# ctu-mrs/mrs_multirotor_simulator

Measured on NVIDIA B200. Metric: UAV-steps/s (RK4+control+collisions) at 1M UAVs, higher is better.
Workload: dtype f64

## Files before the change

mrs_multirotor_simulator_b200/csrc/api.cu:

```cuda
#include <dlfcn.h>
#include <nccl.h>

#include <algorithm>
#include <cmath>
#include <cstdarg>
#include <cstdio>
#include <cstring>
#include <functional>
#include <map>
#include <memory>
#include <string>
#include <type_traits>
#include <utility>
#include <vector>

#include "internal.h"
#include "params.h"

static thread_local char g_err[512] = "";

static int fail(int code, const char* fmt, ...) {
  va_list ap;
  va_start(ap, fmt);
  vsnprintf(g_err, sizeof(g_err), fmt, ap);
// ... 68 lines not shown

  int alloc(size_t count) {
    Mem m;
    if (Pinned) {
      CU(cudaHostAlloc(&m.p_, sizeof(T) * count, cudaHostAllocMapped));
    } else {
      CU(cudaMalloc(&m.p_, sizeof(T) * count));
    }
    m.cap_ = count;
    *this  = std::move(m);
    return MRSB_OK;
  }
  int grow(size_t need, size_t count, cudaStream_t stream) {
    if (need <= cap_) return MRSB_OK;
    Mem m;
    int rc = m.alloc(count);
    if (rc) return rc;
    if (p_) CU(cudaStreamSynchronize(stream));
    *this = std::move(m);
    return MRSB_OK;
  }

 private:
  void release() {
    if (p_) Pinned ? cudaFreeHost(p_) : cudaFree(p_);
  }
  T*     p_   = nullptr;
  size_t cap_ = 0;
};

struct ParamSet {
  mrsb_model_params      mp;
  mrsb_controller_params cp;
};

#define MAX_BUCKETS 8
struct Bucket {
  int64_t   slot0 = 0, count = 0;
  int       nm    = 0;
  int       pset  = -1;
  DevParams params{};
};

static_assert(std::is_trivially_copyable_v<DevState> && std::is_trivially_copyable_v<DevGrid> && std::is_trivially_copyable_v<PeerView> &&
              std::is_trivially_copyable_v<P2PCtl> && std::is_trivially_copyable_v<DevParams> && std::is_trivially_copyable_v<Bucket>);
struct GraphArgs {
  DevState s;
  DevGrid  grid;
  PeerView pv;
  P2PCtl   p2p;
  int32_t  crash, lists;
  double   rebounce;
  int32_t with_step, k_substeps, uniform_mode, any_moment, publish, n_buckets;
  double  dt;
  Bucket  buckets[MAX_BUCKETS];
};
static_assert(std::is_trivially_copyable_v<GraphArgs>);

struct Graph {
  cudaGraphExec_t exec = nullptr;
  int             own  = 0;
  GraphArgs       key{};

  Graph() = default;
  explicit Graph(const GraphArgs& a) { std::memcpy(&key, &a, sizeof(a)); }
  Graph(Graph&& o) noexcept { *this = std::move(o); }
  Graph& operator=(Graph&& o) noexcept {
    if (exec) cudaGraphExecDestroy(exec);
    exec = std::exchange(o.exec, nullptr), own = o.own;
    std::memcpy(&key, &o.key, sizeof(key));
    return *this;
  }
  ~Graph() {
    if (exec) cudaGraphExecDestroy(exec);
  }
  bool holds(const GraphArgs& a) const { return std::memcmp(&key, &a, sizeof(a)) == 0; }
};

struct mrsb_sim {
  int          device = 0;
  cudaStream_t stream = nullptr;
  DevState     ds{};
  DevGrid      grid{};
  Mem<int32_t> pairs;

  std::vector<ParamSet>      sets;
  std::map<std::string, int> set_index;
  std::vector<Mem<unsigned char>> mem;

  std::vector<int32_t>       pset_host;
  Mem<DevParams>             d_params;
  Mem<uint8_t>               d_takeoff0;
  int32_t*                   d_pset       = nullptr;
  bool                       params_dirty = true;

  Mem<char>    d_stage;
  Mem<int32_t> d_idx;

  int  uniform_mode = MRSB_INPUT_UNKNOWN;
  bool any_moment   = false;
  std::vector<Bucket>  buckets;
  std::vector<int32_t> perm_host, inv_host;
  int32_t*             d_perm = nullptr;
  int32_t*             d_inv  = nullptr;

  int    coll_enabled = 0, coll_crash = 0;
  double coll_rebounce = 0.0;

  double   filt_dt  = -1.0;
  uint32_t outputs  = MRSB_OUT_IMU | MRSB_OUT_POSITIONS;
  bool     iterate_without_input = true;
  double*  d_geom[2] = {nullptr, nullptr};

  ncclComm_t           comm    = nullptr;
  int                  n_ranks = 1, rank = 0;
  std::vector<int64_t> shard_begin_of, shard_count_of;
  bool                 equal_shards = true;

  bool                 p2p       = false;
  double*              gbuf[2]   = {nullptr, nullptr};
  uint32_t*            d_gbox[2] = {nullptr, nullptr};
  int64_t              pass_no   = 0;
  bool                 wrote_since_pass = false;
  std::vector<int32_t> pending_geom[2];
  PeerView             pv[2]{};
  PeerView             pv_local{};
  P2PCtl               p2pctl{};
// ... 1152 lines not shown
  if (h->p2p) {
    h->pass_no++;
    const int w         = write_buf(h);
    h->ds.gpos          = h->gbuf[w];
    h->ds.gbox          = h->d_gbox[w];
    h->ds.geom          = h->d_geom[w];
    h->wrote_since_pass = false;
    int rc              = apply_pending_geom(h, w);
    if (rc) return rc;
  }
  CU(cudaGetLastError());
  return MRSB_OK;
}

static int collide_local(mrsb_sim* h) {
  if (h->p2p && !h->wrote_since_pass) {
    h->n_launches += launch_publish_positions(h->ds, h->stream);
    h->wrote_since_pass = true;
  }
  if (h->lists_on) {
    int rc = before_list_pass(h);
    if (rc) return rc;
  } else {
    h->steps_since_pass = 0;
  }
  GraphArgs a;
  graph_args(h, false, 0.0, 0, &a);
  Graph& g       = h->pass[write_buf(h)];
  bool   graphed = !h->graph_failed && !getenv("MRSB_NO_GRAPH");
  if (graphed && !(g.exec && g.holds(a))) {
    g               = build_pass_graph(h, a);
    graphed         = g.exec != nullptr;
    h->graph_failed = !graphed;
  }
  if (graphed) {
    CU(cudaGraphLaunch(g.exec, h->stream));
    h->n_launches += g.own;
  } else if (a.lists) {
    h->n_launches += launch_collide_decide(a.grid, a.p2p, 1, cudaGraphConditionalHandle{}, 0, h->stream);
    h->rebuild_own = launch_collide_rebuild(a.s, a.grid, a.pv, h->stream);
    h->rebuild_own += launch_collide_check(a.s, a.grid, a.pv, a.crash, a.rebounce, 0, h->stream);
  } else {
    h->n_launches += launch_collide(a.s, a.grid, a.pv, a.p2p, a.crash, a.rebounce, h->stream);
  }
  return after_pass(h);
}

static int before_step(mrsb_sim* h, double dt, int32_t k_substeps) {
  if (k_substeps < 1) return fail(MRSB_ERR_INVALID, "k_substeps must be >= 1");
  int rc = flush_params(h);
  if (rc) return rc;
  rc = ensure_filt(h, dt);
  if (rc) return rc;
  if (h->p2p && *h->h_status.get()) return fail(MRSB_ERR_STATE, "peer hand-shake timed out (a rank stopped calling the collision pass)");
  return MRSB_OK;
}

int mrsb_make_step(mrsb_handle h, double dt, int32_t k_substeps) {
  GUARD(h);
  int rc = before_step(h, dt, k_substeps);
  if (rc) return rc;
  GraphArgs a;
  graph_args(h, true, dt, k_substeps, &a);
  h->n_launches += launch_step_buckets(a, h->stream, h->step_info);
  h->wrote_since_pass = true;
  h->n_steps += k_substeps;
  h->steps_since_pass++;
  CU(cudaGetLastError());
  return MRSB_OK;
}

static int before_collisions(mrsb_sim* h) {
  int rc = flush_params(h);
  if (rc) return rc;
  if (h->ds.n_global > h->ds.n && h->n_ranks <= 1) return fail(MRSB_ERR_STATE, "sharded handle without communicator");
  if (h->lists_on && (h->positions_touched || h->steps_since_pass != 1))
    CU(cudaMemcpyAsync(&h->grid.ctl->disp_max_bits, h->h_one.get() + 1, sizeof(uint32_t), cudaMemcpyHostToDevice, h->stream));
  return MRSB_OK;
}

int mrsb_handle_collisions(mrsb_handle h) {
  GUARD(h);
  if (!(h->coll_crash || h->coll_enabled)) return MRSB_OK;
  int rc = before_collisions(h);
  if (rc) return rc;
  rc = exchange_positions(h);
  if (rc) return rc;
  return collide_local(h);
}

int mrsb_handle_collisions_gathered(mrsb_handle h) {
  GUARD(h);
  if (!(h->coll_crash || h->coll_enabled)) return MRSB_OK;
  int rc = flush_params(h);
  if (rc) return rc;
  return collide_local(h);
}

static int run_tick_graph(mrsb_sim* h, double dt, int32_t k_substeps, bool* done) {
  *done = false;
  if (!h->lists_on || h->graph_failed || getenv("MRSB_NO_GRAPH")) return MRSB_OK;
  if (h->positions_touched || h->steps_since_pass != 0) return MRSB_OK;
  GraphArgs a;
  graph_args(h, true, dt, k_substeps, &a);
  Graph& g = h->tick[write_buf(h)];
  if (!g.holds(a)) {
    g = Graph(a);
    return MRSB_OK;
  }
  if (!g.exec) {
    g = build_pass_graph(h, a);
    if (!g.exec) {
      h->graph_failed = true;
      return MRSB_OK;
    }
  }
  h->wrote_since_pass = true;
  h->n_steps += k_substeps;
  h->list_passes++;
  CU(cudaGraphLaunch(g.exec, h->stream));
  h->n_launches += g.own;
  *done = true;
  return after_pass(h);
}

int mrsb_run(mrsb_handle h, double dt, int32_t k_substeps, int32_t n_ticks, int32_t with_collisions) {
  GUARD(h);
  const bool collide = with_collisions && (h->coll_crash || h->coll_enabled);
  for (int t = 0; t < n_ticks; t++) {
    if (collide) {
      int rc = before_step(h, dt, k_substeps);
      if (rc) return rc;
      bool done = false;
      rc        = run_tick_graph(h, dt, k_substeps, &done);
      if (rc) return rc;
      if (done) continue;
    }
    int rc = mrsb_make_step(h, dt, k_substeps);
    if (rc) return rc;
    if (collide) {
      rc = mrsb_handle_collisions(h);
      if (rc) return rc;
    }
  }
  return MRSB_OK;
}

int mrsb_get_state(mrsb_handle h, int64_t n, const int32_t* idx, double* x, double* v, double* R, double* omega, double* motor_rpm) {
  GUARD(h);
  int rc = MRSB_OK;
  if (x && !rc) rc = get_rows(h, h->ds.st, ST_ROWS, 0, 3, n, idx, x);
  if (v && !rc) rc = get_rows(h, h->ds.st, ST_ROWS, 3, 3, n, idx, v);
  if (R && !rc) rc = get_rows(h, h->ds.st, ST_ROWS, 6, 9, n, idx, R);
  if (omega && !rc) rc = get_rows(h, h->ds.st, ST_ROWS, 15, 3, n, idx, omega);
  if (motor_rpm && !rc) rc = get_rows(h, h->ds.rpm, MRSB_NM, 0, MRSB_NM, n, idx, motor_rpm);
  return rc;
}

int mrsb_get_v_prev(mrsb_handle h, int64_t n, const int32_t* idx, double* v_prev) {
  GUARD(h);
  return download(h, n, idx, sizeof(double) * 3 * size_t(n), v_prev, [&](const int32_t* d_idx, void* d_out) {
    return launch_gather_vprev(h->ds, n, d_idx, static_cast<double*>(d_out), h->stream);
  });
}
// ... 749 lines not shown
```

mrs_multirotor_simulator_b200/csrc/collide.cu:

```cuda
#include <algorithm>

#include "internal.h"

namespace {

#define DEV __device__ __forceinline__

#define NL_LIVE 0x80000000u
#define NL_CROWDED 0x40000000u

DEV unsigned long long now_ns() {
  unsigned long long t;
  asm volatile("mov.u64 %0, %globaltimer;" : "=l"(t));
  return t;
}
DEV void stamp(const DevGrid& g, int slot, unsigned long long value) {
  if (g.tl) g.tl[((g.ctl->n_passes - 1ull) % MRSB_TL_TICKS) * 8 + slot] = value;
}

DEV int cell_of(double v, double inv_cell) {
  return __double2int_rd(__dmul_rn(v, inv_cell));
}

DEV uint32_t row_hash(int cy, int cz) {
  uint32_t h = uint32_t(cy) * 0x9E3779B1u ^ (uint32_t(cz) * 0x85EBCA77u + 0x165667B1u);
  h ^= h >> 15;
  h *= 0x2C1B3C6Du;
  h ^= h >> 12;
  return h;
}

DEV unsigned long long enc(double v) {
  const unsigned long long b = (unsigned long long)__double_as_longlong(v);
  return (b >> 63) ? ~b : (b | 0x8000000000000000ull);
}
DEV double dec(unsigned long long e) {
  const unsigned long long b = (e >> 63) ? (e & 0x7fffffffffffffffull) : ~e;
  return __longlong_as_double((long long)b);
}
DEV float fdec(uint32_t e) {
  return __uint_as_float((e >> 31) ? (e & 0x7fffffffu) : ~e);
}

DEV int owner_of(const PeerView& pv, int64_t gj) {
  int r = 0;
  while (r + 1 < pv.n_ranks && gj >= pv.begin[r + 1]) r++;
  return r;
}
DEV void load_pos(const DevState& s, int64_t gj, double& x, double& y, double& z) {
  const double* p = s.gpos + 3 * gj;
  x = p[0], y = p[1], z = p[2];
}
struct Geom {
  double arm, prop, mass;
};
DEV Geom load_geom(const DevState& s, int64_t gj) {
  const double* p = s.geom + 4 * gj;
  Geom          g;
  g.arm = p[0], g.prop = p[1], g.mass = p[2];
  return g;
}

__global__ void box_reset_kernel(unsigned long long* aabb) {
  if (threadIdx.x < 3) aabb[threadIdx.x] = ~0ull;
  if (threadIdx.x >= 3 && threadIdx.x < 6) aabb[threadIdx.x] = 0ull;
}

__global__ void __launch_bounds__(256) box_kernel(const double* __restrict__ gpos, int64_t begin, int64_t n, unsigned long long* aabb) {
// ... 626 lines not shown
          hits &= hits - 1;
        }
      } else {
        int64_t last = -1;
        while (hits) {
          int64_t  best = INT64_MAX;
          uint32_t bc   = 0;
          for (uint32_t m = hits; m; m &= m - 1) {
            const uint32_t c  = uint32_t(__ffs(int(m)) - 1);
            const int64_t  gj = g.act_items[int64_t(c) * g.nl_ld + k];
            if (gj > last && gj < best) best = gj, bc = c;
          }
          if (best == INT64_MAX) break;
          process(bc);
          last = best;
          hits &= ~(1u << bc);
        }
      }
    }
  }
  const bool nz = nonzero(acc);
  if (live || nz) store_result(s, li, acc);
  else if (acc.crashed_me) s.flags[slot_of(s, li)] |= FLAG_CRASHED;
  if (nz != bool(word & NL_LIVE)) {
    const uint32_t nw = (word & ~NL_LIVE) | (nz ? NL_LIVE : 0u);
    g.nl_count[li]    = nw;
    g.nl_active[k].y  = nw;
  }
}

#ifndef MRSB_CHECK_THREADS
#define MRSB_CHECK_THREADS 256
#define MRSB_CHECK_MINB 4
#endif
__global__ void __launch_bounds__(MRSB_CHECK_THREADS, MRSB_CHECK_MINB) check_kernel(DevState s, DevGrid g, int crash_mode, double rebounce, int skip_if_rebuild) {
  if (skip_if_rebuild && g.ctl->rebuild) return;
  if (blockIdx.x == 0 && threadIdx.x == 0) stamp(g, 4, now_ns());
  const uint32_t n_active = g.ctl->n_active;
  for (uint32_t k = blockIdx.x * blockDim.x + threadIdx.x; k < n_active; k += gridDim.x * blockDim.x) {
    const uint2 e = g.nl_active[k];
    int32_t     first4[4];
#pragma unroll
    for (int u = 0; u < 4; u++) first4[u] = g.act_items[int64_t(u) * g.nl_ld + k];
    check_one(s, g, crash_mode, rebounce, k, int64_t(e.x), e.y, first4);
  }
}

__global__ void __launch_bounds__(32) decide_kernel(NlCtl* __restrict__ c, unsigned long long* __restrict__ pair_counter, double skin, int always,
                                                    cudaGraphConditionalHandle handle, int has_handle, P2PCtl p, unsigned long long* tl) {
  const uint32_t full = 0xffffffffu;
  const int      lane = threadIdx.x;
  unsigned long long* row = tl ? tl + (c->n_passes % MRSB_TL_TICKS) * 8 : nullptr;
  if (row && lane == 0) row[0] = now_ns();
  uint32_t                 bits  = c->disp_max_bits;
  const double             D_old = c->D_total;
  const uint32_t           force = c->force, valid = c->valid;
  const unsigned long long n_rebuilds = c->n_rebuilds, n_passes = c->n_passes;
  if (p.n_ranks > 1) {
    const unsigned long long epoch = c->epoch + 1ull;
    const int                slot  = int(epoch & 1ull);
    const bool               peer  = lane < p.n_ranks && lane != p.rank;
    volatile unsigned long long* theirs = peer ? p.peer_flags[lane] : nullptr;
    if (peer) theirs[p.n_ranks + 2 * p.rank + slot] = (unsigned long long)(always ? 0xFFFFFFFFu : bits);
    __threadfence_system();
    if (peer) theirs[p.rank] = epoch;
    if (row && lane == 0) row[1] = now_ns();
    uint32_t got = 0u;
    if (peer) {
      volatile const unsigned long long* mine = p.flags;
      const long long                    t0   = clock64();
      bool                               ok   = true;
      while (mine[lane] < epoch) {
        if (clock64() - t0 > p.budget) {
          *p.status = 1;
          ok        = false;
          break;
        }
        __nanosleep(32);
      }
      __threadfence_system();
      got = ok ? uint32_t(mine[p.n_ranks + 2 * lane + slot]) : 0xFFFFFFFFu;
    }
    bits = max(bits, __reduce_max_sync(full, got));
    if (lane == 0) c->epoch = epoch;
  }
  if (lane != 0) return;
  if (row) row[2] = now_ns();
  const double d       = __dsqrt_ru(double(__uint_as_float(bits)));
  double       D       = __dadd_ru(D_old, d);
  const bool   rebuild = always || force || !valid || !(__dmul_ru(2.0, D) <= skin);
  if (has_handle) cudaGraphSetConditional(handle, rebuild ? 1u : 0u);
  *pair_counter    = 0ull;
  c->disp_max_bits = 0u;
  if (rebuild) {
    D            = 0.0;
    c->force     = 0u;
    c->valid     = 1u;
    c->n_crowded = 0u;
    c->n_active  = 0u;
    c->n_rebuilds = n_rebuilds + 1ull;
  }
  if (row) row[5] = rebuild ? 1ull : 0ull;
  c->D_total  = D;
  c->rebuild  = rebuild ? 1u : 0u;
  c->n_passes = n_passes + 1ull;
}


__global__ void __launch_bounds__(256) nb_pack_kernel(DevState s, double* __restrict__ pos, double* __restrict__ vel) {
  const int64_t i = int64_t(blockIdx.x) * blockDim.x + threadIdx.x;
  if (i >= s.ld) return;
  const int64_t e = s.inv ? int64_t(s.inv[i]) : (i < s.n ? i : -1);
  if (e < 0) return;
#pragma unroll
  for (int c = 0; c < 3; c++) {
    pos[3 * e + c] = s.st[tix(ST_ROWS, c, i)];
    vel[3 * e + c] = s.st[tix(ST_ROWS, 3 + c, i)];
  }
}

DEV bool nb_before(double da, int32_t ja, double db, int32_t jb) { return da < db || (da == db && ja < jb); }

template <int K>
__global__ void __launch_bounds__(128) nb_query_kernel(DevGrid t, int64_t n, const double* __restrict__ pos, const double* __restrict__ vel, double r2,
                                                        int k, int32_t* __restrict__ idx_out, double* __restrict__ rows_out, int64_t stride,
                                                        int32_t* __restrict__ count_out) {
  const int64_t p = int64_t(blockIdx.x) * blockDim.x + threadIdx.x;
  if (p >= n) return;
  const double4 q = t.rec[p];
  const int64_t i = __double_as_longlong(q.w);
  double        bd[K];
  int32_t       bj[K];
#pragma unroll
  for (int u = 0; u < K; u++) bd[u] = __longlong_as_double(0x7FF0000000000000ll), bj[u] = INT32_MAX;
  int32_t cnt = 0;
  if (isfinite(q.x) && isfinite(q.y) && isfinite(q.z)) {
    const Stencil st = stencil_of(t, q.x, q.y, q.z);
    for (int a = 0; a < 4; a++) {
      for (uint32_t r = st.lo[a]; r < st.hi[a]; r++) {
        const double4 c  = t.rec[r];
        const double  d2 = nf_dist2(c.x, c.y, c.z, q.x, q.y, q.z);
        if (!(d2 < r2)) continue;
        const int32_t j = int32_t(__double_as_longlong(c.w));
        if (int64_t(j) == i || cell_of(c.y, t.inv_cell) != st.rcy[a] || cell_of(c.z, t.inv_cell) != st.rcz[a]) continue;
        cnt++;
        if (!nb_before(d2, j, bd[K - 1], bj[K - 1])) continue;
        bd[K - 1] = d2, bj[K - 1] = j;
#pragma unroll
        for (int u = K - 1; u > 0; u--) {
          if (nb_before(bd[u], bj[u], bd[u - 1], bj[u - 1])) {
            const double  td = bd[u];
            const int32_t tj = bj[u];
            bd[u] = bd[u - 1], bj[u] = bj[u - 1];
            bd[u - 1] = td, bj[u - 1] = tj;
          }
        }
      }
    }
// ... 143 lines not shown
```

mrs_multirotor_simulator_b200/csrc/internal.h:

```cpp
#pragma once
#include <cuda_runtime.h>
#include <stdint.h>

#include "../../include/mrsb.h"

#define MRSB_NM MRSB_MAX_MOTORS
#define MRSB_TILE 128

static __host__ __device__ __forceinline__ int64_t tix(int rows, int row, int64_t i) {
  return ((i >> 7) * rows + row) * MRSB_TILE + (i & (MRSB_TILE - 1));
}
#define ST_ROWS 18
#define VPREV_ROWS 3
#define F3_ROWS 3

#define FLAG_CRASHED 1u
#define FLAG_TAKEOFF 2u
#define FLAG_VPREV 4u
#define FLAG_HAD_INPUT 256u
#define FLAG_FF_VEL_HDG_RATE 16u
#define FLAG_FF_VEL_HDG 32u
#define FLAG_FF_ACC_HDG_RATE 64u
#define FLAG_FF_ACC_HDG 128u

// ... 38 lines not shown
  double*  initz;
  double*  cmd;
  double*  ff;
  uint32_t* flags;
  uint8_t*  mode;
  const int32_t* pset;
  const DevParams* params;
  double* geom;
  double*  gpos;
  int64_t  shard_begin;
  int64_t  n_global;
  uint32_t* gbox;
  int64_t   n_groups32;
  int32_t  n_ranks, rank;
  uint32_t opts;
  const int32_t* perm;
  const int32_t* inv;
  uint32_t* disp_max;
};

#define STEP_OPT_IMU 1u
#define STEP_OPT_GPOS 2u
#define STEP_OPT_NEED_INPUT 4u

#define MRSB_MAX_RANKS 16
struct PeerView {
  int32_t         n_ranks, rank;
  int64_t         begin[MRSB_MAX_RANKS + 1];
  const double*   pos[MRSB_MAX_RANKS];
  const uint32_t* box[MRSB_MAX_RANKS];
  const double*   geom[MRSB_MAX_RANKS];
};

struct P2PCtl {
  unsigned long long* const* peer_flags;
  unsigned long long*        flags;
  int32_t                    n_ranks, rank;
  int*                       status;
  long long                  budget;
};

#define MRSB_NL_CAP 8
#define MRSB_TL_TICKS 4096
struct NlCtl {
  uint32_t disp_max_bits;
  uint32_t force;
  uint32_t valid;
  uint32_t n_active;
  uint32_t n_crowded;
  uint32_t rebuild;
  double   D_total;
  unsigned long long n_rebuilds, n_passes, epoch ;
  unsigned long long write_all_until;
};

struct DevGrid {
  uint32_t  n_buckets;
  uint32_t  bits;
  double    inv_cell;
  double    reach;
  double    list_r2;
  double    skin;
  uint32_t* nl_count;
  int32_t*  nl_items;
  int64_t   nl_ld;
  uint2*    nl_active;
  int32_t*  act_items;
  NlCtl*    ctl;
  uint32_t* bucket;
  uint32_t* rank;
  uint32_t* count;
  uint32_t* begin;
  double4*  rec;
  unsigned long long* aabb;
  unsigned long long* scan_state;
  int32_t   scan_tiles;
  double4*  halo_rec;
  uint32_t* halo_bucket, *halo_rank;
  uint32_t* halo_n;
  uint32_t* halo_work;
  uint32_t* halo_work_n;
  int64_t   halo_cap;
  unsigned long long* tl;
  int32_t*  pairs;
  int64_t   pair_cap;
  unsigned long long* counters;
};

int launch_step(const DevState& s, const DevParams* uniform_params, double dt, int k_substeps, int uniform_mode, int uniform_nm, bool any_moment,
                cudaStream_t stream, int* info);
int launch_prep_params(DevParams* params, int n_sets, double dt, cudaStream_t stream);
int launch_collide(const DevState& s, const DevGrid& g, const PeerView& pv, const P2PCtl& p2p, int crash_mode, double rebounce, cudaStream_t stream);
int launch_collide_decide(const DevGrid& g, const P2PCtl& p2p, int always, cudaGraphConditionalHandle handle, int has_handle, cudaStream_t stream);
int launch_collide_rebuild(const DevState& s, const DevGrid& g, const PeerView& pv, cudaStream_t stream);
int launch_collide_check(const DevState& s, const DevGrid& g, const PeerView& pv, int crash_mode, double rebounce, int beside_rebuild, cudaStream_t stream);
int scan_tiles_for(int64_t n_items);
int launch_neighbours(const DevState& s, const DevGrid& t, double* pos, double* vel, double r2, int k, int32_t* idx, double* rows, int stride,
                      int32_t* count, cudaStream_t stream);
int launch_publish_positions(const DevState& s, cudaStream_t stream);

int launch_scatter_input(const DevState& s, int mode, int64_t n, const int32_t* idx_dev, const double* payload_dev, int stride, cudaStream_t stream);
int launch_input_rows(const DevState& s, int64_t n, const int32_t* idx_dev, const int32_t* modes_dev, const double* payload_dev, int stride,
                      int32_t* last_dev, cudaStream_t stream);
int launch_scatter_rows(double* dst, int rows_total, int row0, int rows, int64_t n, const int32_t* idx_dev, const double* payload_dev, int stride,
                        const int32_t* perm, cudaStream_t stream);
int launch_gather_rows(const double* src, int rows_total, int row0, int rows, int64_t n, const int32_t* idx_dev, double* out_dev, int stride,
                       const int32_t* perm, cudaStream_t stream);
int launch_flag_update(const DevState& s, int64_t n, const int32_t* idx_dev, uint32_t and_mask, uint32_t or_mask, cudaStream_t stream);
int launch_gather_u32(const uint32_t* src, int64_t n, const int32_t* idx_dev, uint32_t* out_dev, const int32_t* perm, cudaStream_t stream);
int launch_gather_u8(const uint8_t* src, int64_t n, const int32_t* idx_dev, int32_t* out_dev, const int32_t* perm, cudaStream_t stream);
int launch_set_mode(const DevState& s, int64_t n, const int32_t* idx_dev, int mode, cudaStream_t stream);
int launch_set_state_pos(const DevState& s, int64_t n, const int32_t* idx_dev, const double* xyz_dev, const double* hdg_dev, cudaStream_t stream);
int launch_respawn(const DevState& s, const uint8_t* takeoff0, int64_t n, const int32_t* idx_dev, const double* xyz_dev, const double* hdg_dev,
                   cudaStream_t stream);
int launch_respawn_masked(const DevState& s, const uint8_t* takeoff0, const uint8_t* mask_dev, const double* xyz_dev, const double* hdg_dev,
                          cudaStream_t stream);
#define SNAP_ROWS 88
int launch_snapshot_save(const DevState& s, double* rows, uint32_t* flags, uint8_t* mode, cudaStream_t stream);
int launch_snapshot_restore(const DevState& s, const double* rows, const uint32_t* flags, const uint8_t* mode, int64_t n, const int32_t* idx_dev,
                            const int32_t* src_dev, cudaStream_t stream);
int launch_snapshot_restore_masked(const DevState& s, const double* rows, const uint32_t* flags, const uint8_t* mode, const int32_t* src_dev,
                                   cudaStream_t stream);
int launch_stash_vprev(const DevState& s, int64_t n, const int32_t* idx_dev, cudaStream_t stream);
int launch_gather_vprev(const DevState& s, int64_t n, const int32_t* idx_dev, double* out_dev, cudaStream_t stream);
int launch_reset_pid(const DevState& s, int64_t n, const int32_t* idx_dev, int pid0, int n_pids, cudaStream_t stream);
int launch_timeout_input(const DevState& s, int64_t n, const int32_t* idx_dev, cudaStream_t stream);
int launch_gather_xyz(const double* xyz_dev, int64_t n, const int32_t* idx_dev, double* out_dev, cudaStream_t stream);
int launch_tracker_cmd(const DevState& s, int64_t n, const int32_t* idx_dev, const double* rows_dev, cudaStream_t stream);
int launch_observe(const DevState& s, int what, int64_t n, const int32_t* idx_dev, double* out_dev, int stride, cudaStream_t stream);
int launch_set_pset(int32_t* pset_dev, int64_t n, const int32_t* idx_dev, int64_t offset, const int32_t* values_dev, cudaStream_t stream);
int launch_set_geom(double* geom_dev, int64_t n, const int32_t* idx_dev, int64_t offset, const int32_t* pset_dev, const DevParams* params, cudaStream_t stream);
```

mrs_multirotor_simulator_b200/csrc/step_kernel.cu:

```cuda
#include <cstdlib>

#include "internal.h"

template <int NM_T>
void launch_step_nm(const DevState& s, const DevParams* uniform_params, double dt, int k_substeps, int uniform_mode, bool any_moment, cudaStream_t stream, int* info);

int launch_step(const DevState& s, const DevParams* uniform_params, double dt, int k_substeps, int uniform_mode, int uniform_nm, bool any_moment,
                cudaStream_t stream, int* info) {
  int scratch[4];
  if (!info) info = scratch;
  info[0] = info[1] = info[2] = info[3] = 0;
  if (s.n <= 0) return 0;
  switch (uniform_nm) {
    case 4:
      launch_step_nm<4>(s, uniform_params, dt, k_substeps, uniform_mode, any_moment, stream, info);
      break;
    case 6:
      launch_step_nm<6>(s, uniform_params, dt, k_substeps, uniform_mode, any_moment, stream, info);
      break;
    case 8:
      launch_step_nm<8>(s, uniform_params, dt, k_substeps, uniform_mode, any_moment, stream, info);
      break;
    default:
      launch_step_nm<0>(s, uniform_params, dt, k_substeps, uniform_mode, any_moment, stream, info);
      break;
  }
  return 1;
}

namespace {
__device__ __forceinline__ uint32_t fenc(float f) {
  const uint32_t b = __float_as_uint(f);
  return (b >> 31) ? ~b : (b | 0x80000000u);
}

__global__ void __launch_bounds__(256) publish_positions_kernel(DevState s) {
  const int64_t i      = int64_t(blockIdx.x) * blockDim.x + threadIdx.x;
  const bool    inside = i < s.n;
  double        x = 0.0, y = 0.0, z = 0.0;
  if (inside) {
    const int64_t slot = s.perm ? int64_t(s.perm[i]) : i;
    x          = s.st[tix(ST_ROWS, 0, slot)];
    y          = s.st[tix(ST_ROWS, 1, slot)];
    z          = s.st[tix(ST_ROWS, 2, slot)];
    double* gp = s.gpos + 3 * (s.shard_begin + i);
    gp[0]      = x;
    gp[1]      = y;
    gp[2]      = z;
  }
  if (s.gbox) {
    const uint32_t full = 0xffffffffu;
    uint32_t lo0 = inside ? fenc(__double2float_rd(x)) : 0xFFFFFFFFu, lo1 = inside ? fenc(__double2float_rd(y)) : 0xFFFFFFFFu,
             lo2 = inside ? fenc(__double2float_rd(z)) : 0xFFFFFFFFu;
    uint32_t hi0 = inside ? fenc(__double2float_ru(x)) : 0u, hi1 = inside ? fenc(__double2float_ru(y)) : 0u, hi2 = inside ? fenc(__double2float_ru(z)) : 0u;
    lo0 = __reduce_min_sync(full, lo0);
    lo1 = __reduce_min_sync(full, lo1);
    lo2 = __reduce_min_sync(full, lo2);
    hi0 = __reduce_max_sync(full, hi0);
    hi1 = __reduce_max_sync(full, hi1);
    hi2 = __reduce_max_sync(full, hi2);
    if ((threadIdx.x & 31) == 0 && i < s.n_groups32 * 32) {
      uint32_t* row = s.gbox + 6 * (i >> 5);
      row[0] = lo0, row[1] = lo1, row[2] = lo2, row[3] = hi0, row[4] = hi1, row[5] = hi2;
    }
  }
}

__global__ void prep_params_kernel(DevParams* params, int n_sets, double dt) {
  const int k = blockIdx.x * blockDim.x + threadIdx.x;
  if (k < n_sets) params[k].filt = exp(dt * params[k].neg_inv_tau);
}
}

int launch_prep_params(DevParams* params, int n_sets, double dt, cudaStream_t stream) {
  if (n_sets <= 0) return 0;
  prep_params_kernel<<<(n_sets + 127) / 128, 128, 0, stream>>>(params, n_sets, dt);
  return 1;
}

int launch_publish_positions(const DevState& s, cudaStream_t stream) {
// ... 5 lines not shown
```

mrs_multirotor_simulator_b200/csrc/step_kernel.cuh:

```cuda
#include <cstdlib>
#include <type_traits>

#pragma once
#include "internal.h"

namespace {

#define DEV __device__ __forceinline__

DEV double rsqrt_fast(double x) {
  double y;
  asm("rsqrt.approx.ftz.f64 %0, %1;" : "=d"(y) : "d"(x));
  const double t = x * y;
  const double e = fma(-t, y, 1.0);
  const double p = fma(0.375, e, 0.5);
  return fma(y * e, p, y);
}
DEV double rcp_fast(double b) {
  double r;
  asm("rcp.approx.ftz.f64 %0, %1;" : "=d"(r) : "d"(b));
  const double e = fma(-b, r, 1.0);
  const double p = fma(e, e, e);
  return fma(r, p, r);
}
DEV double sqrt_fast(double x) {
  if (x > 1e-290 && x < 1e300) return x * rsqrt_fast(x);
  return sqrt(x);
}
DEV unsigned expo(double v) { return unsigned(__double2hiint(v)) & 0x7ff00000u; }

struct Vec3 {
  double x, y, z;
};
DEV Vec3 mk(double x, double y, double z) {
  Vec3 r;
  r.x = x;
  r.y = y;
  r.z = z;
  return r;
}
DEV Vec3   operator+(Vec3 a, Vec3 b) { return mk(a.x + b.x, a.y + b.y, a.z + b.z); }
DEV Vec3   operator-(Vec3 a, Vec3 b) { return mk(a.x - b.x, a.y - b.y, a.z - b.z); }
DEV Vec3   operator*(Vec3 a, double s) { return mk(a.x * s, a.y * s, a.z * s); }
DEV double dot(Vec3 a, Vec3 b) { return fma(a.x, b.x, fma(a.y, b.y, a.z * b.z)); }
DEV Vec3   cross(Vec3 a, Vec3 b) { return mk(fma(a.y, b.z, -(a.z * b.y)), fma(a.z, b.x, -(a.x * b.z)), fma(a.x, b.y, -(a.y * b.x))); }
DEV Vec3   fma3(Vec3 a, double s, Vec3 b) { return mk(fma(a.x, s, b.x), fma(a.y, s, b.y), fma(a.z, s, b.z)); }
DEV Vec3 normalized(Vec3 a) {
  const double z = dot(a, a);
  if (z > 1e-290 && z < 1e300) return a * rsqrt_fast(z);
  if (z > 0.0) return a * (1.0 / sqrt(z));
  return a;
}
DEV unsigned expo3(Vec3 a) { return max(expo(a.x), max(expo(a.y), expo(a.z))); }
DEV bool isnan3(Vec3 a) { return (a.x != a.x) | (a.y != a.y) | (a.z != a.z); }
DEV Vec3 nan0(Vec3 a) { return mk(a.x != a.x ? 0.0 : a.x, a.y != a.y ? 0.0 : a.y, a.z != a.z ? 0.0 : a.z); }

struct Rot {
// ... 663 lines not shown
  if ((threadIdx.x & 31) == 0 && disp_bits > *reinterpret_cast<volatile uint32_t*>(s.disp_max)) atomicMax(s.disp_max, disp_bits);
}

template <int NM_T, int MODE_T, bool ONE>
__global__ void __launch_bounds__(MRSB_STEP_THREADS, MRSB_STEP_MINB(ONE, MODE_T))
    uav_step_kernel(DevState s, double dt, double inv_dt, int k_sub, int any_moment) {
  const int64_t tile = blockIdx.x;
  TileIn        in;
  in.st   = s.st + (tile * ST_ROWS) * MRSB_TILE + threadIdx.x;
  in.rpm  = s.rpm + (tile * MRSB_NM) * MRSB_TILE + threadIdx.x;
  in.pid  = s.pid + (tile * PID_ROWS) * MRSB_TILE + threadIdx.x;
  in.cmd  = s.cmd + (tile * CMD_ROWS) * MRSB_TILE + threadIdx.x;
  in.fext = s.fext + (tile * F3_ROWS) * MRSB_TILE + threadIdx.x;
  const int64_t i = min(tile * MRSB_TILE + threadIdx.x, s.n - 1);
  uint32_t disp_bits = 0u;
  step_uav<NM_T, MODE_T, ONE>(s, in, tile, s.flags[i], nullptr, s.pset[s.shard_begin + (s.inv ? int64_t(s.inv[i]) : i)], dt, inv_dt, k_sub, any_moment, disp_bits,
                              [] {});
  report_displacement(s, disp_bits);
}

template <int NM_T, int MODE_T>
struct Img {
  static constexpr int  pid_lo   = MODE_T == MRSB_POSITION_CMD ? 0 : MODE_T >= MRSB_VELOCITY_HDG_RATE_CMD ? 3 : MODE_T >= MRSB_ATTITUDE_CMD ? 6 : MODE_T >= MRSB_ATTITUDE_RATE_CMD ? 9 : 12;
  static constexpr int  cmd_rows = MODE_T == MRSB_ACTUATOR_CMD ? NM_T : MODE_T == MRSB_ATTITUDE_CMD ? 10 : MODE_T == MRSB_TILT_HDG_RATE_CMD ? 5 : 4;
  static constexpr bool hdg      = MODE_T == MRSB_POSITION_CMD || MODE_T == MRSB_VELOCITY_HDG_CMD || MODE_T == MRSB_ACCELERATION_HDG_CMD;
  static constexpr int  ST       = 0;
  static constexpr int  RPM      = ST + ST_ROWS;
  static constexpr int  PID      = RPM + NM_T;
  static constexpr int  CMD      = PID + (pid_lo < 12 ? PID_ROWS - pid_lo : 0);
  static constexpr int  FEXT     = CMD + (hdg ? CMD_ROWS : cmd_rows);
  static constexpr int  ROWS     = FEXT + F3_ROWS;
};

template <int NM_T, int MODE_T>
DEV void stage_tile(const DevState& s, const DevParams& P, double* sm, uint64_t* bar, int64_t tile) {
  static_assert(MODE_T >= 0 && NM_T > 0, "the staged kernel is for batches with a uniform input mode and motor count");
  using I = Img<NM_T, MODE_T>;
  const bool     rate_int = P.rate_ki[0] != 0.0 || P.rate_ki[1] != 0.0 || P.rate_ki[2] != 0.0;
  constexpr int  kRow     = MRSB_TILE * int(sizeof(double));
  constexpr int  pid_lo   = I::pid_lo;
  const int      int_rows = pid_lo < 12 ? (rate_int ? 12 - pid_lo : 9 - pid_lo) : 0;
  const uint32_t bytes    = uint32_t(kRow) * uint32_t(ST_ROWS + NM_T + (12 - pid_lo) + int_rows + I::cmd_rows + (I::hdg ? 2 : 0) + F3_ROWS);
  mbar_expect_tx(bar, bytes);
  tma_load(sm + I::ST * MRSB_TILE, s.st + (tile * ST_ROWS) * MRSB_TILE, kRow * ST_ROWS, bar);
  tma_load(sm + I::RPM * MRSB_TILE, s.rpm + (tile * MRSB_NM) * MRSB_TILE, kRow * NM_T, bar);
  if (pid_lo < 12) tma_load(sm + I::PID * MRSB_TILE, s.pid + (tile * PID_ROWS + pid_lo) * MRSB_TILE, kRow * (12 - pid_lo), bar);
  if (int_rows > 0) tma_load(sm + (I::PID + 12) * MRSB_TILE, s.pid + (tile * PID_ROWS + 12 + pid_lo) * MRSB_TILE, uint32_t(kRow) * uint32_t(int_rows), bar);
  tma_load(sm + I::CMD * MRSB_TILE, s.cmd + (tile * CMD_ROWS) * MRSB_TILE, kRow * I::cmd_rows, bar);
  if (I::hdg) tma_load(sm + (I::CMD + CMD_COS) * MRSB_TILE, s.cmd + (tile * CMD_ROWS + CMD_COS) * MRSB_TILE, kRow * 2, bar);
  tma_load(sm + I::FEXT * MRSB_TILE, s.fext + (tile * F3_ROWS) * MRSB_TILE, kRow * F3_ROWS, bar);
}

template <int NM_T, int MODE_T, bool ONE>
__global__ void __launch_bounds__(MRSB_STEP_THREADS, MRSB_STEP_MINB(ONE, MODE_T))
    uav_step_staged_kernel(DevState s, const __grid_constant__ DevParams params, double dt, double inv_dt, int k_sub, int any_moment, int64_t n_tiles) {
  using I = Img<NM_T, MODE_T>;
  extern __shared__ __align__(128) double sm[];
  __shared__ uint64_t bar;
  if (threadIdx.x == 0) mbar_init(&bar, 1);
  __syncthreads();
  int64_t tile = blockIdx.x;
  if (threadIdx.x == 0 && tile < n_tiles) stage_tile<NM_T, MODE_T>(s, params, sm, &bar, tile);
  TileIn in;
  in.st   = sm + I::ST * MRSB_TILE + threadIdx.x;
  in.rpm  = sm + I::RPM * MRSB_TILE + threadIdx.x;
  in.pid  = sm + (I::PID - I::pid_lo) * MRSB_TILE + threadIdx.x;
  in.cmd  = sm + I::CMD * MRSB_TILE + threadIdx.x;
  in.fext = sm + I::FEXT * MRSB_TILE + threadIdx.x;
  uint32_t phase = 0;
  int64_t  i0        = min(tile * MRSB_TILE + threadIdx.x, s.n - 1);
  uint32_t flags_cur = tile < n_tiles ? s.flags[i0] : 0u;
  uint32_t disp_bits = 0u;
  for (; tile < n_tiles; tile += gridDim.x) {
    const int64_t next = tile + gridDim.x;
    uint32_t      flags_next = 0u;
    if (next < n_tiles) flags_next = s.flags[min(next * MRSB_TILE + threadIdx.x, s.n - 1)];
    mbar_wait(&bar, phase);
    phase ^= 1u;
    step_uav<NM_T, MODE_T, ONE>(
        s, in, tile, flags_cur, &params, 0, dt, inv_dt, k_sub, any_moment, disp_bits,
        [&] {
          __syncthreads();
          if (threadIdx.x == 0 && next < n_tiles) stage_tile<NM_T, MODE_T>(s, params, sm, &bar, next);
        },
        ONE ? nullptr : sm + I::ROWS * MRSB_TILE);
    flags_cur = flags_next;
  }
  report_displacement(s, disp_bits);
}

template <int NM_T, int MODE_T, bool ONE>
int staged_grid(size_t smem) {
  static int cached = -1;
  if (cached < 0) {
    auto* k = uav_step_staged_kernel<NM_T, MODE_T, ONE>;
    if (cudaFuncSetAttribute(k, cudaFuncAttributeMaxDynamicSharedMemorySize, int(smem)) != cudaSuccess) {
      cudaGetLastError();
      cached = 0;
      return cached;
    }
    int dev = 0, sms = 0, per_sm = 0;
    cudaGetDevice(&dev);
    cudaDeviceGetAttribute(&sms, cudaDevAttrMultiProcessorCount, dev);
    cudaOccupancyMaxActiveBlocksPerMultiprocessor(&per_sm, k, MRSB_STEP_THREADS, smem);
    cached = sms * per_sm;
  }
  return cached;
}

template <int NM_T, int MODE_T>
void launch_one(const DevState& s, const DevParams* uniform_params, double dt, int k, int any_moment, cudaStream_t st, int* info) {
  const int     threads = MRSB_STEP_THREADS;
  const int64_t n_tiles = (s.n + threads - 1) / threads;
  const double  inv_dt  = 1.0 / dt;
  info[2] = NM_T;
  info[3] = MODE_T;
  if constexpr (NM_T > 0 && MODE_T >= 0) if (uniform_params && !getenv("MRSB_NO_STAGING")) {
    auto launch = [&](auto one) -> bool {
      constexpr bool kOne = decltype(one)::value;
      const size_t   smem = size_t(Img<NM_T, MODE_T>::ROWS + (kOne ? 0 : PID_ROWS)) * MRSB_TILE * sizeof(double);
      const int      grid = staged_grid<NM_T, MODE_T, kOne>(smem);
      if (grid <= 0 || n_tiles <= grid) return false;
      uav_step_staged_kernel<NM_T, MODE_T, kOne><<<grid, threads, smem, st>>>(s, *uniform_params, dt, inv_dt, k, any_moment, n_tiles);
      info[0] = 2;
      info[1] = grid;
      return true;
    };
    if ((k == 1) ? launch(std::true_type{}) : launch(std::false_type{})) return;
  }
  info[0] = 1;
  info[1] = int(n_tiles);
  if (k == 1) {
    uav_step_kernel<NM_T, MODE_T, true><<<unsigned(n_tiles), threads, 0, st>>>(s, dt, inv_dt, k, any_moment);
  } else {
    uav_step_kernel<NM_T, MODE_T, false><<<unsigned(n_tiles), threads, 0, st>>>(s, dt, inv_dt, k, any_moment);
  }
}

template <int NM_T>
void launch_nm(const DevState& s, const DevParams* up, double dt, int k, int mode, int any_moment, cudaStream_t st, int* info) {
  switch (mode) {
    case MRSB_ACTUATOR_CMD:
      launch_one<NM_T, MRSB_ACTUATOR_CMD>(s, up, dt, k, any_moment, st, info);
      break;
    case MRSB_VELOCITY_HDG_RATE_CMD:
      launch_one<NM_T, MRSB_VELOCITY_HDG_RATE_CMD>(s, up, dt, k, any_moment, st, info);
      break;
    case MRSB_VELOCITY_HDG_CMD:
      launch_one<NM_T, MRSB_VELOCITY_HDG_CMD>(s, up, dt, k, any_moment, st, info);
      break;
    case MRSB_POSITION_CMD:
      launch_one<NM_T, MRSB_POSITION_CMD>(s, up, dt, k, any_moment, st, info);
      break;
    default:
      launch_one<NM_T, -1>(s, up, dt, k, any_moment, st, info);
      break;
  }
}

}

template <int NM_T>
void launch_step_nm(const DevState& s, const DevParams* uniform_params, double dt, int k_substeps, int uniform_mode, bool any_moment, cudaStream_t stream,
                    int* info) {
  launch_nm<NM_T>(s, uniform_params, dt, k_substeps, uniform_mode, any_moment, stream, info);
}
```

mrs_multirotor_simulator_b200/csrc/step_kernel_nm4.cu:

```cuda
#include "step_kernel.cuh"

template void launch_step_nm<4>(const DevState&, const DevParams*, double, int, int, bool, cudaStream_t, int*);
```

mrs_multirotor_simulator_b200/csrc/step_kernel_nm6.cu:

```cuda
#include "step_kernel.cuh"

template void launch_step_nm<6>(const DevState&, const DevParams*, double, int, int, bool, cudaStream_t, int*);
```

mrs_multirotor_simulator_b200/csrc/step_kernel_nm8.cu:

```cuda
#include "step_kernel.cuh"

template void launch_step_nm<8>(const DevState&, const DevParams*, double, int, int, bool, cudaStream_t, int*);
```

Measured before the change: 6.339 billion.

## Fuse step and neighbour-list decide into one tick kernel with device-side rebuild launch

Adds a fused tick kernel: the persistent staged step kernel ends with a last-block-arrives counter barrier, and that block runs the neighbour-list rebuild decision. When a rebuild is needed, it tail-launches a device-launchable rebuild graph instead of going through a separate decide kernel and a conditional graph node. This removes one kernel launch and the conditional-node overhead per tick in the single-rank, uniform-parameter, k=1 case. It adds an atomic barrier, a device graph launch path and a new failure status word to check.

```diff
diff --git a/mrs_multirotor_simulator_b200/csrc/api.cu b/mrs_multirotor_simulator_b200/csrc/api.cu
--- a/mrs_multirotor_simulator_b200/csrc/api.cu
+++ b/mrs_multirotor_simulator_b200/csrc/api.cu
@@ -144,14 +144,16 @@
   int32_t  crash, lists;
   double   rebounce;
   int32_t with_step, k_substeps, uniform_mode, any_moment, publish, n_buckets;
+  int32_t fused;
   double  dt;
   Bucket  buckets[MAX_BUCKETS];
 };
 static_assert(std::is_trivially_copyable_v<GraphArgs>);
 
 struct Graph {
-  cudaGraphExec_t exec = nullptr;
-  int             own  = 0;
+  cudaGraphExec_t exec    = nullptr;
+  cudaGraphExec_t rebuild = nullptr;
+  int             own     = 0;
   GraphArgs       key{};
 
   Graph() = default;
@@ -159,12 +161,14 @@
   Graph(Graph&& o) noexcept { *this = std::move(o); }
   Graph& operator=(Graph&& o) noexcept {
     if (exec) cudaGraphExecDestroy(exec);
-    exec = std::exchange(o.exec, nullptr), own = o.own;
+    if (rebuild) cudaGraphExecDestroy(rebuild);
+    exec = std::exchange(o.exec, nullptr), rebuild = std::exchange(o.rebuild, nullptr), own = o.own;
     std::memcpy(&key, &o.key, sizeof(key));
     return *this;
   }
   ~Graph() {
     if (exec) cudaGraphExecDestroy(exec);
+    if (rebuild) cudaGraphExecDestroy(rebuild);
   }
   bool holds(const GraphArgs& a) const { return std::memcmp(&key, &a, sizeof(a)) == 0; }
 };
@@ -1423,7 +1427,10 @@
   if (rc) return rc;
   rc = ensure_filt(h, dt);
   if (rc) return rc;
-  if (h->p2p && *h->h_status.get()) return fail(MRSB_ERR_STATE, "peer hand-shake timed out (a rank stopped calling the collision pass)");
+  if (const int* st = h->h_status.get()) {
+    if (*st == TICK_STATUS_LAUNCH) return fail(MRSB_ERR_STATE, "status word %d: the tick kernel could not launch the neighbour-list rebuild", *st);
+    if (*st) return fail(MRSB_ERR_STATE, "status word %d: peer hand-shake timed out (a rank stopped calling the collision pass)", *st);
+  }
   return MRSB_OK;
 }
 
@@ -1468,19 +1475,67 @@
   return collide_local(h);
 }
 
+static Graph build_fused_tick(mrsb_sim* h, const GraphArgs& a) {
+  Graph         g(a);
+  const Bucket& b = a.buckets[0];
+  DevState      v = a.s;
+  v.n             = b.count;
+  TickCtl t{};
+  t.g = a.grid;
+  if (launch_tick(v, &b.params, a.dt, a.uniform_mode, b.nm, a.any_moment, t, false, h->stream, nullptr) <= 0) return g;
+  if (!h->h_status.get()) {
+    if (h->h_status.alloc(1) != MRSB_OK) return g;
+    *h->h_status.get() = 0;
+  }
+  t.status = h->h_status.get();
+  cudaStream_t side = nullptr;
+  cudaGraph_t  rebuild = nullptr, tick = nullptr;
+  int          own_rebuild = 0;
+  bool         ok = cudaStreamCreateWithFlags(&side, cudaStreamNonBlocking) == cudaSuccess &&
+            cudaStreamBeginCapture(side, cudaStreamCaptureModeThreadLocal) == cudaSuccess;
+  if (ok) {
+    own_rebuild = launch_collide_rebuild(a.s, a.grid, a.pv, side);
+    own_rebuild += launch_collide_check(a.s, a.grid, a.pv, a.crash, a.rebounce, 0, side);
+    ok = cudaStreamEndCapture(side, &rebuild) == cudaSuccess && rebuild &&
+         cudaGraphInstantiate(&g.rebuild, rebuild, cudaGraphInstantiateFlagDeviceLaunch) == cudaSuccess && cudaGraphUpload(g.rebuild, h->stream) == cudaSuccess;
+  }
+  t.rebuild = g.rebuild;
+  int own = 0;
+  if (ok && cudaStreamBeginCapture(h->stream, cudaStreamCaptureModeThreadLocal) == cudaSuccess) {
+    const bool launched = launch_tick(v, &b.params, a.dt, a.uniform_mode, b.nm, a.any_moment, t, true, h->stream, h->step_info) > 0;
+    own = 1 + launch_collide_check(a.s, a.grid, a.pv, a.crash, a.rebounce, 1, h->stream);
+    ok = cudaStreamEndCapture(h->stream, &tick) == cudaSuccess && tick && launched;
+  } else {
+    ok = false;
+  }
+  ok = ok && cudaGraphInstantiate(&g.exec, tick, cudaGraphInstantiateFlagDeviceLaunch) == cudaSuccess && cudaGraphUpload(g.exec, h->stream) == cudaSuccess;
+  if (rebuild) cudaGraphDestroy(rebuild);
+  if (tick) cudaGraphDestroy(tick);
+  if (side) cudaStreamDestroy(side);
+  cudaGetLastError();
+  if (!ok) return Graph(a);
+  g.own          = own;
+  h->rebuild_own = own_rebuild;
+  return g;
+}
+
 static int run_tick_graph(mrsb_sim* h, double dt, int32_t k_substeps, bool* done) {
   *done = false;
   if (!h->lists_on || h->graph_failed || getenv("MRSB_NO_GRAPH")) return MRSB_OK;
   if (h->positions_touched || h->steps_since_pass != 0) return MRSB_OK;
   GraphArgs a;
   graph_args(h, true, dt, k_substeps, &a);
+  a.fused = h->n_ranks <= 1 && h->ds.n_global == h->ds.n && a.n_buckets == 1 && a.buckets[0].pset >= 0 && a.buckets[0].nm > 0 &&
+            a.buckets[0].slot0 == 0 && a.uniform_mode >= 0 && k_substeps == 1 && !getenv("MRSB_NO_FUSED_TICK");
   Graph& g = h->tick[write_buf(h)];
   if (!g.holds(a)) {
+    if (g.rebuild) CU(cudaStreamSynchronize(h->stream));
     g = Graph(a);
     return MRSB_OK;
   }
   if (!g.exec) {
-    g = build_pass_graph(h, a);
+    if (a.fused) g = build_fused_tick(h, a);
+    if (!g.exec) g = build_pass_graph(h, a);
     if (!g.exec) {
       h->graph_failed = true;
       return MRSB_OK;
diff --git a/mrs_multirotor_simulator_b200/csrc/collide.cu b/mrs_multirotor_simulator_b200/csrc/collide.cu
--- a/mrs_multirotor_simulator_b200/csrc/collide.cu
+++ b/mrs_multirotor_simulator_b200/csrc/collide.cu
@@ -1,6 +1,6 @@
 #include <algorithm>
 
-#include "internal.h"
+#include "nl_decide.cuh"
 
 namespace {
 
@@ -9,11 +9,6 @@
 #define NL_LIVE 0x80000000u
 #define NL_CROWDED 0x40000000u
 
-DEV unsigned long long now_ns() {
-  unsigned long long t;
-  asm volatile("mov.u64 %0, %globaltimer;" : "=l"(t));
-  return t;
-}
 DEV void stamp(const DevGrid& g, int slot, unsigned long long value) {
   if (g.tl) g.tl[((g.ctl->n_passes - 1ull) % MRSB_TL_TICKS) * 8 + slot] = value;
 }
@@ -746,10 +741,8 @@
   const int      lane = threadIdx.x;
   unsigned long long* row = tl ? tl + (c->n_passes % MRSB_TL_TICKS) * 8 : nullptr;
   if (row && lane == 0) row[0] = now_ns();
-  uint32_t                 bits  = c->disp_max_bits;
-  const double             D_old = c->D_total;
-  const uint32_t           force = c->force, valid = c->valid;
-  const unsigned long long n_rebuilds = c->n_rebuilds, n_passes = c->n_passes;
+  uint32_t      bits = c->disp_max_bits;
+  const NlWords w    = nl_words(c);
   if (p.n_ranks > 1) {
     const unsigned long long epoch = c->epoch + 1ull;
     const int                slot  = int(epoch & 1ull);
@@ -780,24 +773,9 @@
   }
   if (lane != 0) return;
   if (row) row[2] = now_ns();
-  const double d       = __dsqrt_ru(double(__uint_as_float(bits)));
-  double       D       = __dadd_ru(D_old, d);
-  const bool   rebuild = always || force || !valid || !(__dmul_ru(2.0, D) <= skin);
+  const bool rebuild = nl_decide(c, pair_counter, w, bits, skin, always);
   if (has_handle) cudaGraphSetConditional(handle, rebuild ? 1u : 0u);
-  *pair_counter    = 0ull;
-  c->disp_max_bits = 0u;
-  if (rebuild) {
-    D            = 0.0;
-    c->force     = 0u;
-    c->valid     = 1u;
-    c->n_crowded = 0u;
-    c->n_active  = 0u;
-    c->n_rebuilds = n_rebuilds + 1ull;
-  }
   if (row) row[5] = rebuild ? 1ull : 0ull;
-  c->D_total  = D;
-  c->rebuild  = rebuild ? 1u : 0u;
-  c->n_passes = n_passes + 1ull;
 }
 
 
diff --git a/mrs_multirotor_simulator_b200/csrc/internal.h b/mrs_multirotor_simulator_b200/csrc/internal.h
--- a/mrs_multirotor_simulator_b200/csrc/internal.h
+++ b/mrs_multirotor_simulator_b200/csrc/internal.h
@@ -114,6 +114,7 @@
   double   D_total;
   unsigned long long n_rebuilds, n_passes, epoch ;
   unsigned long long write_all_until;
+  uint32_t bar_arrive, bar_base;
 };
 
 struct DevGrid {
@@ -152,6 +153,14 @@
 int launch_step(const DevState& s, const DevParams* uniform_params, double dt, int k_substeps, int uniform_mode, int uniform_nm, bool any_moment,
                 cudaStream_t stream, int* info);
 int launch_prep_params(DevParams* params, int n_sets, double dt, cudaStream_t stream);
+#define TICK_STATUS_LAUNCH 2
+struct TickCtl {
+  DevGrid         g;
+  cudaGraphExec_t rebuild;
+  int*            status;
+};
+int launch_tick(const DevState& s, const DevParams* uniform_params, double dt, int uniform_mode, int uniform_nm, bool any_moment, const TickCtl& t,
+                bool launch, cudaStream_t stream, int* info);
 int launch_collide(const DevState& s, const DevGrid& g, const PeerView& pv, const P2PCtl& p2p, int crash_mode, double rebounce, cudaStream_t stream);
 int launch_collide_decide(const DevGrid& g, const P2PCtl& p2p, int always, cudaGraphConditionalHandle handle, int has_handle, cudaStream_t stream);
 int launch_collide_rebuild(const DevState& s, const DevGrid& g, const PeerView& pv, cudaStream_t stream);
diff --git a/mrs_multirotor_simulator_b200/csrc/nl_decide.cuh b/mrs_multirotor_simulator_b200/csrc/nl_decide.cuh
--- /dev/null
+++ b/mrs_multirotor_simulator_b200/csrc/nl_decide.cuh
@@ -0,0 +1,45 @@
+#pragma once
+#include "internal.h"
+
+namespace {
+
+#define DEV __device__ __forceinline__
+
+DEV unsigned long long now_ns() {
+  unsigned long long t;
+  asm volatile("mov.u64 %0, %globaltimer;" : "=l"(t));
+  return t;
+}
+
+struct NlWords {
+  double             D_old;
+  uint32_t           force, valid;
+  unsigned long long n_rebuilds, n_passes;
+};
+DEV NlWords nl_words(const NlCtl* c) {
+  NlWords w;
+  w.D_old = c->D_total, w.force = c->force, w.valid = c->valid, w.n_rebuilds = c->n_rebuilds, w.n_passes = c->n_passes;
+  return w;
+}
+
+DEV bool nl_decide(NlCtl* c, unsigned long long* pair_counter, const NlWords& w, uint32_t bits, double skin, bool always) {
+  const double d       = __dsqrt_ru(double(__uint_as_float(bits)));
+  double       D       = __dadd_ru(w.D_old, d);
+  const bool   rebuild = always || w.force || !w.valid || !(__dmul_ru(2.0, D) <= skin);
+  *pair_counter        = 0ull;
+  c->disp_max_bits     = 0u;
+  if (rebuild) {
+    D             = 0.0;
+    c->force      = 0u;
+    c->valid      = 1u;
+    c->n_crowded  = 0u;
+    c->n_active   = 0u;
+    c->n_rebuilds = w.n_rebuilds + 1ull;
+  }
+  c->D_total  = D;
+  c->rebuild  = rebuild ? 1u : 0u;
+  c->n_passes = w.n_passes + 1ull;
+  return rebuild;
+}
+
+}
diff --git a/mrs_multirotor_simulator_b200/csrc/step_kernel.cu b/mrs_multirotor_simulator_b200/csrc/step_kernel.cu
--- a/mrs_multirotor_simulator_b200/csrc/step_kernel.cu
+++ b/mrs_multirotor_simulator_b200/csrc/step_kernel.cu
@@ -4,6 +4,10 @@
 
 template <int NM_T>
 void launch_step_nm(const DevState& s, const DevParams* uniform_params, double dt, int k_substeps, int uniform_mode, bool any_moment, cudaStream_t stream, int* info);
+
+template <int NM_T>
+int launch_tick_nm(const DevState& s, const DevParams* uniform_params, double dt, int uniform_mode, bool any_moment, const TickCtl& t, bool launch,
+                   cudaStream_t stream, int* info);
 
 int launch_step(const DevState& s, const DevParams* uniform_params, double dt, int k_substeps, int uniform_mode, int uniform_nm, bool any_moment,
                 cudaStream_t stream, int* info) {
@@ -26,6 +30,23 @@
       break;
   }
   return 1;
+}
+
+int launch_tick(const DevState& s, const DevParams* uniform_params, double dt, int uniform_mode, int uniform_nm, bool any_moment, const TickCtl& t,
+                bool launch, cudaStream_t stream, int* info) {
+  int scratch[4];
+  if (!info) info = scratch;
+  if (s.n <= 0) return 0;
+  switch (uniform_nm) {
+    case 4:
+      return launch_tick_nm<4>(s, uniform_params, dt, uniform_mode, any_moment, t, launch, stream, info);
+    case 6:
+      return launch_tick_nm<6>(s, uniform_params, dt, uniform_mode, any_moment, t, launch, stream, info);
+    case 8:
+      return launch_tick_nm<8>(s, uniform_params, dt, uniform_mode, any_moment, t, launch, stream, info);
+    default:
+      return 0;
+  }
 }
 
 namespace {
diff --git a/mrs_multirotor_simulator_b200/csrc/step_kernel.cuh b/mrs_multirotor_simulator_b200/csrc/step_kernel.cuh
--- a/mrs_multirotor_simulator_b200/csrc/step_kernel.cuh
+++ b/mrs_multirotor_simulator_b200/csrc/step_kernel.cuh
@@ -3,6 +3,7 @@
 
 #pragma once
 #include "internal.h"
+#include "nl_decide.cuh"
 
 namespace {
 
@@ -772,8 +773,7 @@
 }
 
 template <int NM_T, int MODE_T, bool ONE>
-__global__ void __launch_bounds__(MRSB_STEP_THREADS, MRSB_STEP_MINB(ONE, MODE_T))
-    uav_step_staged_kernel(DevState s, const __grid_constant__ DevParams params, double dt, double inv_dt, int k_sub, int any_moment, int64_t n_tiles) {
+DEV uint32_t step_tiles(const DevState& s, const DevParams& params, double dt, double inv_dt, int k_sub, int any_moment, int64_t n_tiles) {
   using I = Img<NM_T, MODE_T>;
   extern __shared__ __align__(128) double sm[];
   __shared__ uint64_t bar;
@@ -806,15 +806,41 @@
         ONE ? nullptr : sm + I::ROWS * MRSB_TILE);
     flags_cur = flags_next;
   }
-  report_displacement(s, disp_bits);
+  return disp_bits;
 }
 
 template <int NM_T, int MODE_T, bool ONE>
-int staged_grid(size_t smem) {
+__global__ void __launch_bounds__(MRSB_STEP_THREADS, MRSB_STEP_MINB(ONE, MODE_T))
+    uav_step_staged_kernel(DevState s, const __grid_constant__ DevParams params, double dt, double inv_dt, int k_sub, int any_moment, int64_t n_tiles) {
+  report_displacement(s, step_tiles<NM_T, MODE_T, ONE>(s, params, dt, inv_dt, k_sub, any_moment, n_tiles));
+}
+
+template <int NM_T, int MODE_T>
+__global__ void __launch_bounds__(MRSB_STEP_THREADS, MRSB_STEP_MINB(true, MODE_T))
+    uav_tick_staged_kernel(DevState s, const __grid_constant__ DevParams params, double dt, double inv_dt, int any_moment, int64_t n_tiles,
+                           const __grid_constant__ TickCtl t) {
+  report_displacement(s, step_tiles<NM_T, MODE_T, true>(s, params, dt, inv_dt, 1, any_moment, n_tiles));
+  __threadfence();
+  __syncthreads();
+  if (threadIdx.x != 0) return;
+  NlCtl* const   c      = t.g.ctl;
+  const uint32_t base   = *reinterpret_cast<volatile uint32_t*>(&c->bar_base);
+  const uint32_t ticket = atomicAdd(&c->bar_arrive, 1u);
+  if (ticket - base != gridDim.x - 1u) return;
+  __threadfence();
+  unsigned long long* row = t.g.tl ? t.g.tl + (c->n_passes % MRSB_TL_TICKS) * 8 : nullptr;
+  if (row) row[0] = now_ns();
+  const bool rebuild = nl_decide(c, t.g.counters, nl_words(c), *reinterpret_cast<volatile uint32_t*>(&c->disp_max_bits), t.g.skin, false);
+  if (row) row[5] = rebuild ? 1ull : 0ull;
+  if (rebuild && cudaGraphLaunch(t.rebuild, cudaStreamGraphTailLaunch) != cudaSuccess) *t.status = TICK_STATUS_LAUNCH;
+  c->bar_base = ticket + 1u;
+}
+
+template <auto K>
+int resident_grid(size_t smem) {
   static int cached = -1;
   if (cached < 0) {
-    auto* k = uav_step_staged_kernel<NM_T, MODE_T, ONE>;
-    if (cudaFuncSetAttribute(k, cudaFuncAttributeMaxDynamicSharedMemorySize, int(smem)) != cudaSuccess) {
+    if (cudaFuncSetAttribute(K, cudaFuncAttributeMaxDynamicSharedMemorySize, int(smem)) != cudaSuccess) {
       cudaGetLastError();
       cached = 0;
       return cached;
@@ -822,10 +848,14 @@
     int dev = 0, sms = 0, per_sm = 0;
     cudaGetDevice(&dev);
     cudaDeviceGetAttribute(&sms, cudaDevAttrMultiProcessorCount, dev);
-    cudaOccupancyMaxActiveBlocksPerMultiprocessor(&per_sm, k, MRSB_STEP_THREADS, smem);
+    cudaOccupancyMaxActiveBlocksPerMultiprocessor(&per_sm, K, MRSB_STEP_THREADS, smem);
     cached = sms * per_sm;
   }
   return cached;
+}
+template <int NM_T, int MODE_T, bool ONE>
+int staged_grid(size_t smem) {
+  return resident_grid<uav_step_staged_kernel<NM_T, MODE_T, ONE>>(smem);
 }
 
 template <int NM_T, int MODE_T>
@@ -857,6 +887,39 @@
   }
 }
 
+template <int NM_T, int MODE_T>
+int tick_one(const DevState& s, const DevParams* uniform_params, double dt, int any_moment, const TickCtl& t, bool launch, cudaStream_t st, int* info) {
+  if constexpr (NM_T > 0 && MODE_T >= 0) {
+    if (!uniform_params || getenv("MRSB_NO_STAGING")) return 0;
+    const int64_t n_tiles = (s.n + MRSB_STEP_THREADS - 1) / MRSB_STEP_THREADS;
+    const size_t  smem    = size_t(Img<NM_T, MODE_T>::ROWS) * MRSB_TILE * sizeof(double);
+    const int     staged  = staged_grid<NM_T, MODE_T, true>(smem);
+    if (staged <= 0 || n_tiles <= staged) return 0;
+    const int grid = resident_grid<uav_tick_staged_kernel<NM_T, MODE_T>>(smem);
+    if (grid <= 0 || !launch) return grid;
+    uav_tick_staged_kernel<NM_T, MODE_T><<<grid, MRSB_STEP_THREADS, smem, st>>>(s, *uniform_params, dt, 1.0 / dt, any_moment, n_tiles, t);
+    info[0] = 2, info[1] = grid, info[2] = NM_T, info[3] = MODE_T;
+    return grid;
+  }
+  return 0;
+}
+
+template <int NM_T>
+int tick_nm(const DevState& s, const DevParams* up, double dt, int mode, int any_moment, const TickCtl& t, bool launch, cudaStream_t st, int* info) {
+  switch (mode) {
+    case MRSB_ACTUATOR_CMD:
+      return tick_one<NM_T, MRSB_ACTUATOR_CMD>(s, up, dt, any_moment, t, launch, st, info);
+    case MRSB_VELOCITY_HDG_RATE_CMD:
+      return tick_one<NM_T, MRSB_VELOCITY_HDG_RATE_CMD>(s, up, dt, any_moment, t, launch, st, info);
+    case MRSB_VELOCITY_HDG_CMD:
+      return tick_one<NM_T, MRSB_VELOCITY_HDG_CMD>(s, up, dt, any_moment, t, launch, st, info);
+    case MRSB_POSITION_CMD:
+      return tick_one<NM_T, MRSB_POSITION_CMD>(s, up, dt, any_moment, t, launch, st, info);
+    default:
+      return 0;
+  }
+}
+
 template <int NM_T>
 void launch_nm(const DevState& s, const DevParams* up, double dt, int k, int mode, int any_moment, cudaStream_t st, int* info) {
   switch (mode) {
@@ -885,3 +948,8 @@
                     int* info) {
   launch_nm<NM_T>(s, uniform_params, dt, k_substeps, uniform_mode, any_moment, stream, info);
 }
+template <int NM_T>
+int launch_tick_nm(const DevState& s, const DevParams* uniform_params, double dt, int uniform_mode, bool any_moment, const TickCtl& t, bool launch,
+                   cudaStream_t stream, int* info) {
+  return tick_nm<NM_T>(s, uniform_params, dt, uniform_mode, any_moment, t, launch, stream, info);
+}
diff --git a/mrs_multirotor_simulator_b200/csrc/step_kernel_nm4.cu b/mrs_multirotor_simulator_b200/csrc/step_kernel_nm4.cu
--- a/mrs_multirotor_simulator_b200/csrc/step_kernel_nm4.cu
+++ b/mrs_multirotor_simulator_b200/csrc/step_kernel_nm4.cu
@@ -1,3 +1,4 @@
 #include "step_kernel.cuh"
 
 template void launch_step_nm<4>(const DevState&, const DevParams*, double, int, int, bool, cudaStream_t, int*);
+template int launch_tick_nm<4>(const DevState&, const DevParams*, double, int, bool, const TickCtl&, bool, cudaStream_t, int*);
diff --git a/mrs_multirotor_simulator_b200/csrc/step_kernel_nm6.cu b/mrs_multirotor_simulator_b200/csrc/step_kernel_nm6.cu
--- a/mrs_multirotor_simulator_b200/csrc/step_kernel_nm6.cu
+++ b/mrs_multirotor_simulator_b200/csrc/step_kernel_nm6.cu
@@ -1,3 +1,4 @@
 #include "step_kernel.cuh"
 
 template void launch_step_nm<6>(const DevState&, const DevParams*, double, int, int, bool, cudaStream_t, int*);
+template int launch_tick_nm<6>(const DevState&, const DevParams*, double, int, bool, const TickCtl&, bool, cudaStream_t, int*);
diff --git a/mrs_multirotor_simulator_b200/csrc/step_kernel_nm8.cu b/mrs_multirotor_simulator_b200/csrc/step_kernel_nm8.cu
--- a/mrs_multirotor_simulator_b200/csrc/step_kernel_nm8.cu
+++ b/mrs_multirotor_simulator_b200/csrc/step_kernel_nm8.cu
@@ -1,3 +1,4 @@
 #include "step_kernel.cuh"
 
 template void launch_step_nm<8>(const DevState&, const DevParams*, double, int, int, bool, cudaStream_t, int*);
+template int launch_tick_nm<8>(const DevState&, const DevParams*, double, int, bool, const TickCtl&, bool, cudaStream_t, int*);
```

Result: slower. 6.276 billion (median of 6 runs) (-1.0%).
